# cuulee/reporter

Measured on AMD Instinct MI355X. Metric: GPS probes matched/sec (whole node), higher is better.
Workload: dtype f64; 1 GPU; c2; graph=metro, nodes=1048576, directed_edges=3527937, osmlr_segments=1361487, traces_per_gpu=10000, streams=1, device_batches=1, output_segments=1688548

## Files before the change

### reporter_amd/csrc/otr_kernels.h

```cpp
#pragma once
#include <cstddef>
#include <type_traits>

#include "otr_device.h"
#include "otr_mincode.h"
#include "otr_report.h"

#ifndef OTR_CAP1
#define OTR_CAP1 160
#endif
#ifndef OTR_LOAD1
#define OTR_LOAD1 7
#endif
#ifndef OTR_E1CAP
#define OTR_E1CAP 360
#endif
#ifndef OTR_E1LOAD
#define OTR_E1LOAD 14
#endif

namespace otr {

struct BatchDev {
  int32_t n_traces;
  const int64_t* trace_off;
  const double* lat;
  const double* lon;
  const int64_t* time;
  const float* acc;
  const uint8_t* mode;
};

__global__ void k_select_states(BatchDev b, ModeParams mp, int64_t* state_cnt, const int64_t* state_off,
                                int64_t* state_probe, int32_t* state_trace) {
  int t = blockIdx.x * blockDim.x + threadIdx.x;
  if (t >= b.n_traces) return;
  const int64_t lo = b.trace_off[t], hi = b.trace_off[t + 1];
  const MatchParams& P = mp.m[b.mode[t] < OTR_MODES ? b.mode[t] : 0];
  int64_t cnt = 0;
  int64_t base = state_off ? state_off[t] : 0;
  double la_last = 0.0, lo_last = 0.0;
  double la_n = lo < hi ? b.lat[lo] : 0.0, lo_n = lo < hi ? b.lon[lo] : 0.0;
  for (int64_t i = lo; i < hi; ++i) {
    const double la = la_n, lg = lo_n;
    if (i + 1 < hi) {
      la_n = b.lat[i + 1];
      lo_n = b.lon[i + 1];
    }
    const bool st = (i == lo || i == hi - 1) || gc_dist(la_last, lo_last, la, lg) >= P.interpolation_distance;
    if (st) {
      if (state_off) {
        state_probe[base + cnt] = i;
        state_trace[base + cnt] = t;
      }
      ++cnt;
      la_last = la;
      lo_last = lg;
    }
// ... 42 lines not shown
    const double by = (e6(pb.x) - plat) * kMetersPerDeg;
    const double dx = bx - ax, dy = by - ay;
    const double l2 = dx * dx + dy * dy;
    double t = 0.0;
    if (l2 > 0.0) {
      t = -(ax * dx + ay * dy) / l2;
      if (t < 0.0) t = 0.0;
      if (t > 1.0) t = 1.0;
    }
    const double qx = ax + t * dx, qy = ay + t * dy;
    const double d2 = qx * qx + qy * qy;
    const double sl = sqrt(l2);
    if (d2 < best) {
      best = d2;
      best_along = acc + t * sl;
      bqx = qx;
      bqy = qy;
    }
    acc = acc + sl;
    pa = pb;
  }
  *tests += k1 - k0 - 1;
  if (!(best <= r2)) return false;
  const double slat = plat + bqy / kMetersPerDeg, slon = plon + bqx / mpl;
  *sr_out = (int64_t)floor((slat - g.grid_min_lat) / g.grid_cell_deg);
  *sc_out = (int64_t)floor((slon - g.grid_min_lon) / g.grid_cell_deg);
  *d2_out = best;
  *frac_out = acc > 0.0 ? best_along / acc : 0.0;
  return true;
}

__device__ inline uint32_t wave_sum_u32(uint32_t v) {
  v += (uint32_t)__builtin_amdgcn_update_dpp(0, (int)v, 0x111, 0xf, 0xf, false);
  v += (uint32_t)__builtin_amdgcn_update_dpp(0, (int)v, 0x112, 0xf, 0xf, false);
  v += (uint32_t)__builtin_amdgcn_update_dpp(0, (int)v, 0x114, 0xf, 0xf, false);
  v += (uint32_t)__builtin_amdgcn_update_dpp(0, (int)v, 0x118, 0xf, 0xf, false);
  v += (uint32_t)__builtin_amdgcn_update_dpp(0, (int)v, 0x142, 0xa, 0xf, false);
  v += (uint32_t)__builtin_amdgcn_update_dpp(0, (int)v, 0x143, 0xc, 0xf, false);
  return (uint32_t)__builtin_amdgcn_readlane((int)v, 63);
}

__device__ inline uint32_t wave_min_u32(uint32_t v) {
  const int I = -1;
  auto mn = [](uint32_t a, int b) { return a < (uint32_t)b ? a : (uint32_t)b; };
  v = mn(v, __builtin_amdgcn_update_dpp(I, (int)v, 0x111, 0xf, 0xf, false));
  v = mn(v, __builtin_amdgcn_update_dpp(I, (int)v, 0x112, 0xf, 0xf, false));
  v = mn(v, __builtin_amdgcn_update_dpp(I, (int)v, 0x114, 0xf, 0xf, false));
  v = mn(v, __builtin_amdgcn_update_dpp(I, (int)v, 0x118, 0xf, 0xf, false));
  v = mn(v, __builtin_amdgcn_update_dpp(I, (int)v, 0x142, 0xa, 0xf, false));
  v = mn(v, __builtin_amdgcn_update_dpp(I, (int)v, 0x143, 0xc, 0xf, false));
  return (uint32_t)__builtin_amdgcn_readlane((int)v, 63);
}

template <int G>
struct Grp {
  static constexpr int GL = OTR_WAVE / G;
  __device__ static int g() { return G == 1 ? 0 : (int)threadIdx.x / GL; }
  __device__ static int gl() { return G == 1 ? (int)threadIdx.x : (int)threadIdx.x % GL; }
  __device__ static unsigned long long mine(unsigned long long m) {
    return G == 1 ? m : (m >> (GL * g())) & ((1ull << GL) - 1ull);
  }
  __device__ static int prefix(unsigned long long m) {
    if (G == 1) return prefix_count(m);
    return __popcll(mine(m) & ((1ull << gl()) - 1ull));
  }
  __device__ static int count(unsigned long long m) { return __popcll(mine(m)); }
  __device__ static int umax(int v) {
    if (G == 1) return __builtin_amdgcn_readfirstlane(v);
    if (G == 8) {
      int m = __builtin_amdgcn_readlane(v, 0);
#pragma unroll
      for (int q = 1; q < 8; ++q) {
        const int x = __builtin_amdgcn_readlane(v, q * GL);
        m = x > m ? x : m;
      }
      return m;
    }
    const int a = __builtin_amdgcn_readlane(v, 0), b = __builtin_amdgcn_readlane(v, GL);
    if (G == 2) return a > b ? a : b;
    const int c = __builtin_amdgcn_readlane(v, 2 * GL), d = __builtin_amdgcn_readlane(v, 3 * GL);
    const int ab = a > b ? a : b, cd = c > d ? c : d;
    return ab > cd ? ab : cd;
  }
  __device__ static bool all(bool v) {
    if (G == 1) return __builtin_amdgcn_readfirstlane((int)v) != 0;
    if (G == 8) {
      bool r = true;
#pragma unroll
      for (int q = 0; q < 8; ++q) r = r && __builtin_amdgcn_readlane((int)v, q * GL) != 0;
      return r;
    }
    const bool ab = __builtin_amdgcn_readlane((int)v, 0) != 0 && __builtin_amdgcn_readlane((int)v, GL) != 0;
    if (G == 2) return ab;
    return ab && __builtin_amdgcn_readlane((int)v, 2 * GL) != 0 && __builtin_amdgcn_readlane((int)v, 3 * GL) != 0;
  }
  __device__ static uint32_t min_u32(uint32_t v) {
    if (G == 1) return wave_min_u32(v);
    if (G == 8) {
#pragma unroll
      for (int o = 1; o < 8; o <<= 1) {
        const uint32_t x = (uint32_t)__shfl_xor((int)v, o, 8);
        v = x < v ? x : v;
      }
      return v;
    }
    const int I = -1;
    auto mn = [](uint32_t a, int b) { return a < (uint32_t)b ? a : (uint32_t)b; };
    v = mn(v, __builtin_amdgcn_update_dpp(I, (int)v, 0x111, 0xf, 0xf, false));
    v = mn(v, __builtin_amdgcn_update_dpp(I, (int)v, 0x112, 0xf, 0xf, false));
    v = mn(v, __builtin_amdgcn_update_dpp(I, (int)v, 0x114, 0xf, 0xf, false));
    v = mn(v, __builtin_amdgcn_update_dpp(I, (int)v, 0x118, 0xf, 0xf, false));
    if (G == 4) {
      const uint32_t a = (uint32_t)__builtin_amdgcn_readlane((int)v, 15);
      const uint32_t b = (uint32_t)__builtin_amdgcn_readlane((int)v, 31);
      const uint32_t c = (uint32_t)__builtin_amdgcn_readlane((int)v, 47);
      const uint32_t d = (uint32_t)__builtin_amdgcn_readlane((int)v, 63);
      const int q = g();
      return q == 0 ? a : (q == 1 ? b : (q == 2 ? c : d));
    }
    v = mn(v, __builtin_amdgcn_update_dpp(I, (int)v, 0x142, 0xa, 0xf, false));
    const uint32_t a = (uint32_t)__builtin_amdgcn_readlane((int)v, 31);
    const uint32_t b = (uint32_t)__builtin_amdgcn_readlane((int)v, 63);
    return g() ? b : a;
  }
};

constexpr int kWin = 16;
#ifndef OTR_CAND2_WAVES
#define OTR_CAND2_WAVES 5
#endif

template <int G>
__global__ __launch_bounds__(64) __attribute__((amdgpu_waves_per_eu(G == 2 ? OTR_CAND2_WAVES : 8, 8))) void k_candidates(
    DevGraph g, BatchDev b, ModeParams mp, int64_t n_states, const int64_t* state_probe, const int32_t* state_trace,
    CandBuf out, unsigned long long* counters) {
  using Gr = Grp<G>;
  constexpr int GL = Gr::GL;
  constexpr int LB = 2 * GL;
  __shared__ double s_d2[G][LB];
  __shared__ double s_p[G][LB];
  __shared__ uint32_t s_e[G][LB];
  __shared__ uint32_t s_bnd[G][kWin][kWin + 1];
  __shared__ uint32_t s_pre[G][kWin + 1];
  const int gi = Gr::g(), lane = Gr::gl();
  const int64_t n_units = (n_states + G - 1) / G;
  const int64_t s = xcd_remap(blockIdx.x, (n_units + 7) / 8) * G + gi;
  if (Gr::umax(s < n_states ? 1 : 0) == 0) return;
// ... 236 lines not shown
  return (m >> (GL * gi)) & ((1ull << GL) - 1ull);
}

template <int LM>
struct LabelT {
  using T = uint32_t;
  using W = uint32_t;
  static constexpr T kInf = 0xFFFFFFFFu;
  static constexpr W kNone = 0xFFFFFFFFu;
  __device__ static W label(T x) { return x; }
  __device__ static T make(W l, uint32_t) { return l; }
};
template <>
struct LabelT<1> {
  using T = unsigned long long;
  using W = uint32_t;
  static constexpr T kInf = 0xFFFFFFFFFFFFFFFFull;
  static constexpr W kNone = 0xFFFFFFFFu;
  __device__ static W label(T x) { return (uint32_t)(x >> 32); }
  __device__ static T make(W l, uint32_t e) { return ((unsigned long long)l << 32) | e; }
};
template <>
struct LabelT<2> {
  using T = unsigned long long;
  using W = unsigned long long;
  static constexpr T kInf = 0xFFFFFFFFFFFFFFFFull;
  static constexpr W kNone = 0xFFFFFFFFFFFFFFFFull;
  __device__ static W label(T x) { return x; }
  __device__ static T make(W l, uint32_t) { return l; }
};

template <class W>
struct WorkE {
  uint32_t node;
  W lab;
};


#ifndef OTR_PCAP1024
#define OTR_PCAP1024 512
#endif
#ifndef OTR_PCAP2048
#define OTR_PCAP2048 512
#endif
#ifndef OTR_PCAP448
#define OTR_PCAP448 448
#endif
#ifndef OTR_WCAP1024
#define OTR_WCAP1024 120
#endif
#ifndef OTR_WCAP4
#define OTR_WCAP4 16
#endif
template <int CAP, int LM>
struct SearchLds {
  static constexpr bool PRED = LM == 1;
  static constexpr bool MI8 = CAP >= 384 && CAP <= 1024 && !PRED;
  using MiT = typename std::conditional<MI8, uint8_t, uint16_t>::type;
  __device__ static MiT code(uint32_t m) {
    if constexpr (MI8) return mf8_of(m);
    else return mi_of(m);
  }
  __device__ static uint32_t gap(MiT c) {
    if constexpr (MI8) return mf8_gap(c);
    else return in_gap(c);
  }
  using W = typename LabelT<LM>::W;
  typename LabelT<LM>::T lab[CAP];
  uint32_t key[CAP];
  MiT mi[CAP];
  using Idx = typename std::conditional<(CAP <= 256 && !PRED), uint8_t, uint16_t>::type;
  static constexpr int WCAP = CAP <= 48 ? 8 : CAP <= 96 ? (PRED ? 20 : OTR_WCAP4) : CAP <= 160 ? 48 : (PRED ? CAP / 4 : (CAP <= 512 ? 64 : (CAP <= 1024 ? OTR_WCAP1024 : 128)));
  static constexpr int PCAP = PRED ? CAP
                                    : (CAP == 1024 ? OTR_PCAP1024 : (CAP == 2048 ? OTR_PCAP2048 : (CAP == 448 ? OTR_PCAP448 : CAP)));
  Idx pend[PCAP];
  WorkE<W> work[WCAP];
  int n_pend, n_keys, overflow;
};

constexpr uint32_t kEmpty = 0xFFFFFFFFu;

constexpr uint32_t kInq = 0x80000000u;
constexpr uint32_t kRel = 0x40000000u;
constexpr uint32_t kNodeMask = 0x0FFFFFFFu;
constexpr uint32_t kNoLabel = 0xFFFFFFFFu;
constexpr uint32_t kNoRoute = 0xFFFFFFFFu;

#ifdef OTR_STAMPS
#define OTR_STAMP(v) unsigned long long v = __builtin_amdgcn_s_memtime()
#else
#define OTR_STAMP(v) const unsigned long long v = 0
#endif

__device__ inline int64_t bound_mm_of(double bound) { return (int64_t)floor(bound * 1000.0); }
__device__ inline int64_t part_mm(double frac, uint32_t len_mm) { return (int64_t)llround(frac * (double)len_mm); }

template <int CAP>
__device__ inline uint32_t hslot(uint32_t node) {
  static_assert(CAP < (1 << 16), "table size fits the 16-bit scale");
  uint32_t p;
  asm("v_mul_u32_u24 %0, %1, %2" : "=v"(p) : "s"(0x9E3779u), "v"(node));
  const uint32_t h = (p >> 8) & 0xFFFFu;
  return __umul24(h, (uint32_t)CAP) >> 16;
}

template <int CAP, int LM>
__device__ inline int lds_find(const SearchLds<CAP, LM>& L, uint32_t node) {
  uint32_t h = hslot<CAP>(node);
  for (int probe = 0; probe < CAP; ++probe) {
    const uint32_t k = L.key[h];
    if (k == kEmpty) return -1;
    if ((k & kNodeMask) == node) return (int)h;
    h = h + 1 == (uint32_t)CAP ? 0u : h + 1;
  }
  return -1;
}

template <int CAP, int LM, bool COUNT = true>
__device__ inline int lds_insert(SearchLds<CAP, LM>& L, uint32_t node, bool* isnew) {
  uint32_t h = hslot<CAP>(node);
  for (int probe = 0; probe < CAP; ++probe) {
    const uint32_t k = atomicCAS(&L.key[h], kEmpty, node);
    if (k == kEmpty) {
      if (COUNT) atomicAdd(&L.n_keys, 1);
      *isnew = true;
      return (int)h;
    }
    if ((k & kNodeMask) == node) {
      *isnew = false;
      return (int)h;
    }
    h = h + 1 == (uint32_t)CAP ? 0u : h + 1;
  }
  L.overflow = 1;
  *isnew = false;
  return -1;
}

template <int CAP, int LM, int G = 1>
__device__ inline void search_init(SearchLds<CAP, LM>* Ls) {
  for (int q = 0; q < G; ++q) {
    SearchLds<CAP, LM>& L = Ls[q];
    for (int k = threadIdx.x; k < CAP; k += OTR_WAVE) {
      L.key[k] = kEmpty;
      L.lab[k] = LabelT<LM>::kInf;
    }
    if (threadIdx.x == 0) {
      L.n_pend = 0;
      L.n_keys = 0;
      L.overflow = 0;
    }
  }
  __syncthreads();
}

struct Pack {
  uint32_t sh;
  __device__ uint32_t tcap() const { return (1u << sh) - 1u; }
  template <class W>
  __device__ uint32_t d(W w) const { return (uint32_t)(w >> sh); }
  template <class W>
  __device__ uint32_t t(W w) const { return (uint32_t)(w & (W)tcap()); }
};
__host__ __device__ inline uint32_t pack_shift(int32_t bt) {
  if (bt < 0) return 0u;
  uint32_t sh = 0;
  while (((1u << sh) - 1u) < (uint32_t)bt + 1u) ++sh;
  return sh;
}
__host__ __device__ inline bool pack_fits(uint32_t bmm, uint32_t sh) {
  return (((uint64_t)bmm << sh) | ((1ull << sh) - 1ull)) < 0xFFFFFFFFull;
}

template <int CAP, int LM>
__device__ inline bool target_resolved(const SearchLds<CAP, LM>& L, const Pack& K, int tslot, uint32_t tpart,
                                       uint32_t gapT, uint32_t pd, uint32_t kmin, bool pend_empty) {
  const int ts = tslot < 0 ? 0 : tslot;
  const uint32_t key = L.key[ts];
  const typename LabelT<LM>::W lw = LabelT<LM>::label(L.lab[ts]);
  const int64_t lab = lw == LabelT<LM>::kNone ? INT64_MAX / 4 : (int64_t)K.d(lw);
  const int64_t next = (int64_t)kmin + (int64_t)gapT;
  const bool unreach = (lab < next ? lab : next) + (int64_t)tpart > (int64_t)pd;
  return (tslot < 0) | pend_empty | ((key & kRel) != 0u) | (lab < next) | unreach;
}

template <int CAP, int LM, bool COUNT = true>
__device__ inline int relax_one(SearchLds<CAP, LM>& L, const Pack& K, uint32_t dw, uint32_t len_mm,
                                uint32_t time_ds, uint32_t minin, typename LabelT<LM>::W pu, uint32_t edge,
                                uint32_t pd, uint32_t pt, uint32_t mode_bit, uint32_t& relaxed, uint32_t& knext,
                                bool& isnew) {
  using W = typename LabelT<LM>::W;
  isnew = false;
  if (!(((dw >> 28) & 7u) & mode_bit)) return -1;
  ++relaxed;
  const uint32_t nd = K.d(pu) + len_mm;
  if (nd > pd) return -1;
  const uint32_t tt = K.t(pu) + time_ds;
  if (tt > pt) return -1;
  const W nw = ((W)nd << K.sh) | (W)tt;
  const int sl = lds_insert<CAP, LM, COUNT>(L, dw & kAdjDstMask, &isnew);
  if (sl < 0) return -1;
  if (isnew) L.mi[sl] = SearchLds<CAP, LM>::code(minin);
  const typename LabelT<LM>::T nb = LabelT<LM>::make(nw, edge);
  const typename LabelT<LM>::T old = atomicMin(&L.lab[sl], nb);
  if (LabelT<LM>::label(nb) < LabelT<LM>::label(old)) {
    knext = nd < knext ? nd : knext;
    const uint32_t ok = atomicOr(&L.key[sl], kInq);
    if (!(ok & kInq)) return sl;
  }
  return -1;
}

template <int CAP>
__device__ inline int relax_sink(SearchLds<CAP, 0>& L, uint32_t* sink, const Pack& K, uint32_t dw, uint32_t len_mm,
                                 uint32_t time_ds, uint32_t minin, uint32_t pu, uint32_t pd, uint32_t pt,
                                 uint32_t mode_bit, uint32_t& relaxed, uint32_t& knext, bool& isnew) {
  const bool mode_ok = (((dw >> 28) & 7u) & mode_bit) != 0u;
  relaxed += mode_ok ? 1u : 0u;
  const uint32_t nd = K.d(pu) + len_mm;
  const uint32_t tt = K.t(pu) + time_ds;
  const uint32_t nw = (nd << K.sh) | tt;
  const uint32_t node = dw & kAdjDstMask;
  bool go = mode_ok && nd <= pd && tt <= pt;
  uint32_t* mine = sink + lane_id();
  const uint32_t h0 = hslot<CAP>(node);
  const uint32_t k0 = atomicCAS(go ? &L.key[h0] : mine, kEmpty, node);
  isnew = go && k0 == kEmpty;
  int sl = (go && (k0 == kEmpty || (k0 & kNodeMask) == node)) ? (int)h0 : -1;
  const bool coll = go && sl < 0;
  if (__ballot(coll) != 0ull) {
    if (coll) {
      uint32_t hh = h0;
      for (int probe = 1; probe < CAP; ++probe) {
        hh = hh + 1 == (uint32_t)CAP ? 0u : hh + 1;
        const uint32_t k = atomicCAS(&L.key[hh], kEmpty, node);
        if (k == kEmpty) {
          isnew = true;
          sl = (int)hh;
          break;
        }
        if ((k & kNodeMask) == node) {
          sl = (int)hh;
          break;
        }
      }
      if (sl < 0) L.overflow = 1;
    }
  }
  go = go && sl >= 0;
  using MiT = typename SearchLds<CAP, 0>::MiT;
  *((go && isnew) ? &L.mi[sl] : reinterpret_cast<MiT*>(mine)) = SearchLds<CAP, 0>::code(minin);
  const uint32_t old = atomicMin(go ? &L.lab[sl] : mine, nw);
  const bool imp = go && nw < old;
  knext = (imp && nd < knext) ? nd : knext;
  const uint32_t was = atomicOr(imp ? &L.key[sl] : mine, kInq);
  return (imp && !(was & kInq)) ? sl : -1;
}

struct NDump {
  const unsigned long long* in;
  unsigned long long* base;
  unsigned long long* ctr;
  uint32_t words, slots;
#ifdef OTR_FORCE_RETRY
  int stop_rounds;
#endif
};
__host__ __device__ constexpr uint32_t nd_words(int cap) { return 2u + (uint32_t)cap + ((uint32_t)cap + 1u) / 2u; }
#ifndef OTR_ND_IN_MIN
#define OTR_ND_IN_MIN 2048
#endif
#ifndef OTR_ND_OUT_MIN
#define OTR_ND_OUT_MIN 1024
#endif

template <int CAP, int LM, int G = 1, bool RIN = false, bool ROUT = false>
__device__ bool search_run(SearchLds<CAP, LM>* Ls, const DevGraph& g, const Pack& K, uint32_t mode_bit, bool active,
                           uint32_t start, uint32_t pd, uint32_t pt, uint32_t tnode, uint32_t tpart, uint32_t gapT,
                           int n_tgt, unsigned long long* settled, unsigned long long* relaxed,
                           unsigned long long* rounds, unsigned long long* stamps = nullptr, uint32_t* sink = nullptr,
                           const NDump* nd = nullptr, int* dslot = nullptr) {
  using Gr = Grp<G>;
  constexpr int kMaxKeys = (CAP <= 128 || CAP >= 256) ? (CAP * 7) / 8 : (CAP * OTR_LOAD1) / 8;
  const int gl = Gr::gl();
  using W = typename LabelT<LM>::W;
  SearchLds<CAP, LM>& L = Ls[Gr::g()];
  using Idx = typename SearchLds<CAP, LM>::Idx;
  constexpr int WCAP = SearchLds<CAP, LM>::WCAP;
  const bool timed = K.sh != 0u;
  const uint32_t* adjt = g.adj_t + (size_t)__builtin_ctz(mode_bit) * g.adj_t_stride;
  uint32_t kmin = 0;
  int npend = active ? 1 : 0;
  const bool resume = RIN && LM == 0 && active && nd->in != nullptr;
  const int nres = resume ? (int)nd->in[0] : 0;
  const int nrx = RIN ? Gr::umax(nres) : 0;
  if (RIN && nrx > 0) {
    const unsigned long long* D = nd->in;
    const uint32_t* M = (const uint32_t*)(D + 2 + nres);
    int np = 0;
    for (int base = 0; base < nrx; base += Gr::GL) {
      const int k = base + gl;
      bool pend = false;
      int sl = 0;
      if (k < nres) {
        const unsigned long long e = D[2 + k];
        const uint32_t key = (uint32_t)(e >> 32), node = key & kNodeMask;
        uint32_t h = hslot<CAP>(node);
        for (int probe = 0; probe < CAP; ++probe) {
          if (atomicCAS(&L.key[h], kEmpty, node) == kEmpty) break;
          h = h + 1 == (uint32_t)CAP ? 0u : h + 1;
        }
        sl = (int)h;
        L.key[sl] = key;
        L.lab[sl] = (typename LabelT<LM>::T)(uint32_t)e;
        L.mi[sl] = SearchLds<CAP, LM>::code(M[k]);
        pend = (key & kInq) != 0u;
      }
      const unsigned long long mp = __ballot(pend);
      if (pend && np + Gr::prefix(mp) < SearchLds<CAP, LM>::PCAP) L.pend[np + Gr::prefix(mp)] = (Idx)sl;
      np += Gr::count(mp);
    }
    if (resume && np > SearchLds<CAP, LM>::PCAP) {
      if (gl == 0) L.overflow = 1;
      np = SearchLds<CAP, LM>::PCAP;
    }
    if (resume) {
      npend = np;
      kmin = (uint32_t)D[1];
      if (gl == 0) L.n_keys = nres;
    }
  }
  if (!resume && active && gl == 0) {
    bool isnew;
    const int sl = lds_insert(L, start, &isnew);
    L.mi[sl] = 0;
    L.lab[sl] = LabelT<LM>::make(0u, kEmpty);
    L.key[sl] |= kInq;
    L.pend[0] = (Idx)sl;
  }
  __syncthreads();
  int tslot = -1;
  if (active && gl < n_tgt && tnode != kEmpty) {
    bool isnew;
    tslot = lds_insert(L, tnode, &isnew);
    if (tslot >= 0 && isnew) L.mi[tslot] = SearchLds<CAP, LM>::code(gapT);
  }
  __syncthreads();
  uint32_t my_settled = 0, my_relaxed = 0, my_rounds = 0;
  unsigned long long cyc[4] = {0, 0, 0, 0};
  bool done = !active, grew = false;
#ifdef OTR_FORCE_RETRY
  int force_round = 0;
#endif
  int nkeys = 0;
  for (;;) {
    OTR_STAMP(t0);
    const int np = done ? 0 : npend;
    OTR_STAMP(t1);
    const bool res = done | (gl >= n_tgt) | target_resolved(L, K, tslot, tpart, gapT, pd, kmin, np == 0);
    done = done || Gr::mine(__ballot(!res)) == 0ull || np == 0;
    OTR_STAMP(t2);
    cyc[0] += t1 - t0;
    cyc[1] += t2 - t1;
    if (Gr::all(done)) break;
    if (!done && gl == 0) ++my_rounds;
    uint32_t knext = 0xFFFFFFFFu;
    int kept = 0, nw = 0;
    const int npx = Gr::umax(np);
    for (int base = 0; base < npx; base += Gr::GL) {
      const int k = base + gl;
      const bool in = k < np;
      const int sl = in ? (int)L.pend[k] : 0;
      const W lb = LabelT<LM>::label(L.lab[sl]);
      const uint32_t key = L.key[sl];
      const uint32_t d = K.d(lb);
      bool take = in && (uint64_t)d < (uint64_t)kmin + SearchLds<CAP, LM>::gap(L.mi[sl]);
      take = take && nw + Gr::prefix(__ballot(take)) < WCAP;
      const unsigned long long mt = __ballot(take), mk = __ballot(in && !take);
      __syncthreads();
      if (take) {
        const uint32_t node = key & kNodeMask;
        L.work[nw + Gr::prefix(mt)] = WorkE<W>{node, lb};
        L.key[sl] = node | kRel;
      }
      const bool keep = in && !take;
      if (keep) L.pend[kept + Gr::prefix(mk)] = (Idx)sl;
      knext = (keep && d < knext) ? d : knext;
      nw += Gr::count(mt);
      kept += Gr::count(mk);
      __syncthreads();
    }
    npend = kept;
    OTR_STAMP(t3);
    cyc[2] += t3 - t2;
    const int nwx = Gr::umax(4 * nw);
    uint32_t tail = 0u;
    for (int base = 0; base < nwx; base += Gr::GL) {
      const int k = base + gl;
      int psl = -1;
      bool isnew = false;
      if (k < 4 * nw) {
        const WorkE<W> wk = L.work[k >> 2];
        const uint32_t wnode = wk.node;
        const int slot = k & 3;
        if (slot == 0) ++my_settled;
        const uint32_t tq = adjt[4 * (size_t)wnode + slot];
        const uint4 r = ld16(g.adj + 4 * (size_t)wnode + slot);
        const uint32_t tt = timed ? tq : 0u;
        if constexpr (LM == 0) {
#ifdef OTR_NO_SINK
          psl = relax_one<CAP, LM, false>(L, K, r.x & ~kAdjMore, r.y, tt, r.z, wk.lab, 0u, pd, pt, mode_bit,
                                          my_relaxed, knext, isnew);
#else
          psl = relax_sink<CAP>(L, sink, K, r.x & ~kAdjMore, r.y, tt, r.z, wk.lab, pd, pt, mode_bit, my_relaxed,
                                knext, isnew);
#endif
        } else {
          const uint32_t e0 = LM == 1 ? g.node_row[wnode] : 0u;
          psl = relax_one<CAP, LM, false>(L, K, r.x & ~kAdjMore, r.y, tt, r.z, wk.lab, e0 + slot, pd, pt, mode_bit,
                                          my_relaxed, knext, isnew);
        }
        tail |= slot == 3 ? (r.x & kAdjMore) : 0u;
      }
      nkeys += Gr::count(__ballot(isnew));
      const unsigned long long mp = __ballot(psl >= 0);
#ifndef OTR_NO_SINK
      if constexpr (LM == 0 && G == 1) {
        const int p = npend + Gr::prefix(mp);
        constexpr int PC = SearchLds<CAP, LM>::PCAP;
        *(psl >= 0 ? &L.pend[p < PC ? p : PC - 1] : reinterpret_cast<Idx*>(sink + lane_id())) = (Idx)psl;
      } else
#endif
      if (psl >= 0) {
        const int p = npend + Gr::prefix(mp);
        L.pend[p < SearchLds<CAP, LM>::PCAP ? p : SearchLds<CAP, LM>::PCAP - 1] = (Idx)psl;
      }
      npend += Gr::count(mp);
    }
    if (SearchLds<CAP, LM>::PCAP < CAP && npend > SearchLds<CAP, LM>::PCAP) {
      if (gl == 0) L.overflow = 1;
      npend = SearchLds<CAP, LM>::PCAP;
    }
    if (__ballot(tail != 0u) != 0ull) {
      if (gl == 0) L.n_pend = npend;
      __syncthreads();
      for (int base = 0; base < nwx; base += Gr::GL) {
        const int k = base + gl;
        if (k < 4 * nw && (k & 3) == 3) {
          const WorkE<W> wk = L.work[k >> 2];
          const uint32_t wnode = wk.node;
          if (g.adj[4 * (size_t)wnode + 3].x & kAdjMore)
            for (uint32_t e = g.node_row[wnode] + 4; e < g.node_row[wnode + 1]; ++e) {
              const uint4 pk = ld16(g.edge_pack + e);
              const uint32_t tt = timed ? g.et(__builtin_ctz(mode_bit))[e] : 0u;
              bool isnew;
              const int psl = relax_one(L, K, pk.x | ((pk.z & 7u) << 28), pk.y, tt, pk.w, wk.lab, e, pd, pt, mode_bit,
                                        my_relaxed, knext, isnew);
              if (psl >= 0) {
                const int p = atomicAdd(&L.n_pend, 1);
                if (p < SearchLds<CAP, LM>::PCAP) L.pend[p] = (Idx)psl;
                else L.overflow = 1;
              }
            }
        }
      }
      __syncthreads();
      npend = L.n_pend;
      if (npend > SearchLds<CAP, LM>::PCAP) npend = SearchLds<CAP, LM>::PCAP;
    }
    __syncthreads();
    OTR_STAMP(t4);
    cyc[3] += t4 - t3;
    const uint32_t km = Gr::min_u32(knext);
    if (!done) kmin = km;
    const int keys = L.n_keys + nkeys;
    if (!done && (L.overflow || keys > kMaxKeys)) {
      grew = !L.overflow && keys > kMaxKeys;
      done = true;
    }
#ifdef OTR_FORCE_RETRY
    ++force_round;
    if (ROUT && !done && nd->base != nullptr && nd->stop_rounds > 0 && force_round >= nd->stop_rounds &&
        !L.overflow) {
      grew = true;
      done = true;
    }
#endif
    __syncthreads();
    if (done && active && gl == 0 && (keys > kMaxKeys || grew)) L.overflow = 1;
  }
  if (gl == 0) L.n_keys += nkeys;
  if (ROUT) *dslot = -1;
  if (ROUT && LM == 0 && __ballot(grew && active && nd->base != nullptr) != 0ull) {
    int v = 0;
    if (grew && active && nd->base != nullptr && gl == 0) v = (int)atomicAdd(nd->ctr, 1ull);
    v = __shfl(v, 0, Gr::GL);
    const bool dump = grew && active && nd->base != nullptr && (uint32_t)v < nd->slots;
    unsigned long long* D = dump ? nd->base + (size_t)v * nd->words : nullptr;
    int n = 0;
    for (int base = 0; base < CAP; base += Gr::GL) {
      const int k = base + gl;
      const uint32_t key = (dump && k < CAP) ? L.key[k] : kEmpty;
      const bool has = key != kEmpty;
      const unsigned long long m = __ballot(has);
      if (has) D[2 + n + Gr::prefix(m)] = (unsigned long long)(uint32_t)L.lab[k] | ((unsigned long long)key << 32);
      n += Gr::count(m);
    }
    uint32_t* M = dump ? (uint32_t*)(D + 2 + n) : nullptr;
    int q = 0;
    for (int base = 0; base < CAP; base += Gr::GL) {
      const int k = base + gl;
      const bool has = dump && k < CAP && L.key[k] != kEmpty;
      const unsigned long long m = __ballot(has);
      if (has) M[q + Gr::prefix(m)] = SearchLds<CAP, LM>::gap(L.mi[k]);
      q += Gr::count(m);
    }
    if (dump && gl == 0) {
      D[0] = (unsigned long long)(uint32_t)n;
      D[1] = kmin;
    }
    *dslot = dump ? v : -1;
  }
#ifdef OTR_STAMPS
  if (stamps && threadIdx.x == 0)
    for (int q = 0; q < 4; ++q) atomicAdd(&stamps[q * kCShards + cshard()], cyc[q]);
#endif
  if (settled) *settled += my_settled;
  if (relaxed) *relaxed += my_relaxed;
  if (rounds) *rounds += my_rounds;
  __syncthreads();
  return !L.overflow;
}

struct PrepArgs {
  int64_t n_states;
  const int64_t* prev;
  const double* bound;
  const int32_t* cand_count;
  const uint32_t* cand_edge;
  const double* cand_p;
  const int32_t* state_trace;
  const uint8_t* mode;
  uint4* cprep;
  uint2* cprep_t;
  uint2* clen;
  int32_t* nroot;
  uint32_t turn_modes;
};

template <int G>
__global__ __launch_bounds__(256) void k_prep(DevGraph g, PrepArgs a) {
  constexpr int GL = OTR_WAVE / G;
  const int64_t s = ((int64_t)blockIdx.x * (blockDim.x / OTR_WAVE) + threadIdx.x / OTR_WAVE) * G +
                    (threadIdx.x % OTR_WAVE) / GL;
  const int lane = threadIdx.x % GL;
  if (s >= a.n_states) return;
  const int K = a.cand_count[s];
  if (K <= 0) return;
// ... 185 lines not shown
  const int32_t bt = a.bt[s];
  const uint32_t sh = pack_shift(bt);
#ifdef OTR_FORCE_GENERAL
  const bool general = true;
#else
  const bool general = !pack_fits(bmm, sh) || turn;
#endif
  uint32_t pre = 0u;
  if (a.est_first_keys > 0 && !general && !turn && !a.forced[s]) {
    float reach = (float)bmm * 1e-3f;
    if (bt >= 0) reach = fminf(reach, (float)bt * 0.1f * a.est_v[md]);
    const float est = a.est_k * reach * reach;
    if (est > (float)a.est_first_keys) {
      uint32_t st = 0;
      while ((int)st + 1 < a.n_tiers && (float)a.tier_keys[st] < est) ++st;
      pre = 1u | (st << 1);
    }
  }
  const uint32_t meta = (uint32_t)a.cand_count[s] | ((uint32_t)md << 8) | ((a.forced[s] ? 1u : 0u) << 10) |
                        (sh << 11) | ((general ? 1u : 0u) << 16) | (turn << 17) | (pre << 18);
  const int64_t to = a.trans_off[s];
  if (turn && a.flag_turn) a.flag_turn[o] = 5;
  a.rec[3 * o] = make_uint4((uint32_t)s, (uint32_t)sp, root, bmm);
  a.rec[3 * o + 1] = make_uint4(d0min, meta, (uint32_t)same, (uint32_t)(same >> 32));
  a.rec[3 * o + 2] = make_uint4(0u, (uint32_t)bt, (uint32_t)to, (uint32_t)((uint64_t)to >> 32));
}

#ifndef OTR_ROUTE2_WAVES
#define OTR_ROUTE2_WAVES 8
#endif

__device__ inline int nth_set_bit(unsigned long long m, int q) {
  for (int j = 0; j < q; ++j) m &= m - 1;
  return __ffsll((long long)m) - 1;
}

template <int CAP, int G, bool LIST, bool WIDE = false, bool CNT = true>
__device__ __forceinline__ void route_unit(const DevGraph& gr, const RouteArgs& a, unsigned long long* counters,
                                           SearchLds<CAP, WIDE ? 2 : 0>* Ls, int64_t w, int64_t n_tasks,
                                           uint32_t* sink, uint4 (*trec)[3]) {
  constexpr int LM = WIDE ? 2 : 0;
  using Gr = Grp<G>;
  const int lane = Gr::gl();
  const int64_t tw = (LIST ? 0 : a.task_base) + w * G + Gr::g();
  const bool have = tw < n_tasks;
  const int64_t task = have ? (LIST ? a.task_list[tw] : tw) : 0;
  OTR_STAMP(ts_in);
  bool search, fits, forced;
  int start_tier = -1;
  uint32_t tnode = kEmpty, tpart = 0, gapT = 1, d0min = 0xFFFFFFFFu, root = 0, bmm = 0, mode_bit = 1;
  uint32_t pd = 0, pt = 0xFFFFFFFFu;
  int Kb;
  Pack K;
  {
    const uint4 r0 = have ? a.rec[3 * task] : make_uint4(0u, 0u, 0u, 0u);
    const uint4 r1 = have ? a.rec[3 * task + 1] : make_uint4(0xFFFFFFFFu, 0u, 0u, 0u);
    const uint4 r2 = have ? a.rec[3 * task + 2] : make_uint4(0u, 0u, 0u, 0u);
    if (lane == 0) {
      trec[Gr::g()][0] = r0;
      trec[Gr::g()][1] = r1;
      trec[Gr::g()][2] = r2;
    }
    const int64_t s = r0.x;
    const unsigned long long mask = ((unsigned long long)r1.w << 32) | r1.z;
    const int64_t sp = r0.y;
    Kb = (int)(r1.y & 0xFFu);
    K.sh = (r1.y >> 11) & 31u;
    const bool general = (r1.y >> 16) & 1u;
    fits = Kb <= Gr::GL && (WIDE || !general) && !((r1.y >> 17) & 1u);
    const bool pre = G >= 2 && !LIST && have && ((r1.y >> 18) & 1u);
    if (pre) {
      start_tier = (int)((r1.y >> 19) & 7u);
      fits = false;
    }
    mode_bit = 1u << ((r1.y >> 8) & 3u);
    bmm = r0.w;
    root = r0.z;
    d0min = r1.x;
    const int32_t bt = (int32_t)r2.y;
    uint32_t ej = 0;
    double pj = 0;
    bool needed = false;
    uint4 cq = make_uint4(0u, 0u, 0u, 0u);
    if (have && !pre && lane < Kb) {
      ej = a.cand_edge[s * OTR_KMAX + lane];
      pj = a.cand_p[s * OTR_KMAX + lane];
      cq = a.cprep[s * OTR_KMAX + lane];
      tpart = cq.x;
    }
    const int nsrc = have && !pre ? __popcll(mask) : 0;
    const int iq = lane < nsrc ? nth_set_bit(mask, lane) : 0;
    uint32_t e_q = 0, t_q = 0;
    double p_q = 0;
    if (lane < nsrc) {
      e_q = a.cand_edge[sp * OTR_KMAX + iq];
      p_q = a.cand_p[sp * OTR_KMAX + iq];
      if (bt >= 0) t_q = a.cprep_t[sp * OTR_KMAX + iq].y;
    }
    for (int q = 0; q < nsrc; ++q) {
      uint32_t ei;
      double pi;
      if (q < Gr::GL) {
        ei = (uint32_t)__shfl((int)e_q, q, Gr::GL);
        pi = __shfl(p_q, q, Gr::GL);
      } else {
        const int i = nth_set_bit(mask, q);
        ei = a.cand_edge[sp * OTR_KMAX + i];
        pi = a.cand_p[sp * OTR_KMAX + i];
      }
      if (lane < Kb && !(ej == ei && pj >= pi)) needed = true;
    }
    const uint32_t t0 = (uint32_t)__shfl((int)t_q, 0, Gr::GL);
    bool feasible_root = d0min <= bmm;
    pd = feasible_root ? bmm - d0min : 0u;
    if (bt >= 0) {
      feasible_root = feasible_root && t0 <= (uint32_t)bt;
      pt = t0 <= (uint32_t)bt ? (uint32_t)bt - t0 : 0u;
    }
    forced = have && ((r1.y >> 10) & 1u);
    const unsigned long long need_mask = __ballot(needed);
    search = have && fits && !forced && feasible_root && Gr::mine(need_mask) != 0ull;
    if (needed) {
      tnode = cq.y;
      gapT = cq.z ? cq.z : 1u;
    }
  }
  unsigned long long settled = 0, relaxed = 0, rounds = 0;
  OTR_STAMP(ts_set);
  NDump nd{};
  int dslot = -1;
  constexpr bool kIn = LIST && !WIDE && CAP >= OTR_ND_IN_MIN, kOut = LIST && !WIDE && CAP >= OTR_ND_OUT_MIN;
  constexpr bool kDumps = kIn || kOut;
  if (kIn) {
    const int32_t rs = (a.dump_in != nullptr && search) ? a.task_dump[task] : -1;
    nd.in = rs >= 0 ? a.dump_in + (size_t)rs * a.dump_in_words : nullptr;
  }
  if (kOut) {
    nd.base = a.dump_out;
    nd.ctr = a.dump_ctr;
    nd.words = a.dump_out_words;
    nd.slots = a.dump_out_slots;
#ifdef OTR_FORCE_RETRY
    nd.stop_rounds = (a.force_edge >> 7) & 1 ? 2 + Gr::g() : 0;
#endif
  }
  search_init<CAP, LM, G>(Ls);
  bool ok = search_run<CAP, LM, G, kIn, kOut>(Ls, gr, K, mode_bit, search, root, pd, pt, tnode, tpart, gapT, Kb, &settled,
                                   &relaxed, &rounds, counters ? counters + 16 * kCShards : nullptr, sink,
                                   kDumps ? &nd : nullptr, kDumps ? &dslot : nullptr) &&
            fits;
#ifdef OTR_FORCE_RETRY
  if (G >= 2 && !LIST) ok = false;
#endif
  OTR_STAMP(ts_srch);
  SearchLds<CAP, LM>& L = Ls[Gr::g()];
  int64_t lab = -1;
  if (ok && search && tnode != kEmpty && !forced) {
    const int sl = lds_find(L, tnode);
    if (sl >= 0 && LabelT<LM>::label(L.lab[sl]) != LabelT<LM>::kNone) lab = (int64_t)LabelT<LM>::label(L.lab[sl]);
  }
  asm volatile("" ::: "memory");
  uint32_t ntr = 0;
  if (have && forced && Kb > Gr::GL) {
    const uint4 r1 = trec[Gr::g()][1], r2 = trec[Gr::g()][2];
    const unsigned long long mask = ((unsigned long long)r1.w << 32) | r1.z;
    uint32_t* trow = a.trans + (int64_t)(((uint64_t)r2.w << 32) | r2.z);
    for (int q = 0; q < __popcll(mask); ++q) {
      const int i = nth_set_bit(mask, q);
      for (int j = lane; j < Kb; j += Gr::GL) trow[(int64_t)i * Kb + j] = kNoRoute;
    }
  } else if (have && (ok || forced)) {
    const uint4 r0 = trec[Gr::g()][0], r1 = trec[Gr::g()][1], r2 = trec[Gr::g()][2];
    const int64_t s = r0.x;
    const unsigned long long mask = ((unsigned long long)r1.w << 32) | r1.z;
    if (search) ntr = (uint32_t)Kb * (uint32_t)__popcll(mask);
    const int64_t sp = r0.y;
    const int32_t bt = (int32_t)r2.y;
    uint32_t* trow = a.trans + (int64_t)(((uint64_t)r2.w << 32) | r2.z);
    const int nsrc = __popcll(mask);
    const int iq = lane < nsrc ? nth_set_bit(mask, lane) : 0;
    uint32_t e_q = 0, w_q = 0, t_q = 0;
    uint2 l_q = make_uint2(0u, 0u);
    double p_q = 0;
    if (lane < nsrc) {
      e_q = a.cand_edge[sp * OTR_KMAX + iq];
      p_q = a.cand_p[sp * OTR_KMAX + iq];
      w_q = a.cprep[sp * OTR_KMAX + iq].w;
      if (bt >= 0) t_q = a.cprep_t[sp * OTR_KMAX + iq].y;
      l_q = a.clen[sp * OTR_KMAX + iq];
    }
    uint32_t ej = 0, tpt = 0;
    double pj = 0;
    if (lane < Kb) {
      ej = a.cand_edge[s * OTR_KMAX + lane];
      pj = a.cand_p[s * OTR_KMAX + lane];
      tpt = bt >= 0 ? a.cprep_t[s * OTR_KMAX + lane].x : 0u;
    }
    for (int q = 0; q < nsrc; ++q) {
      int i;
      uint32_t ei, wi, ti, li, lti;
      double pi;
      if (q < Gr::GL) {
        i = __shfl(iq, q, Gr::GL);
        ei = (uint32_t)__shfl((int)e_q, q, Gr::GL);
        pi = __shfl(p_q, q, Gr::GL);
        wi = (uint32_t)__shfl((int)w_q, q, Gr::GL);
        ti = (uint32_t)__shfl((int)t_q, q, Gr::GL);
        li = (uint32_t)__shfl((int)l_q.x, q, Gr::GL);
        lti = (uint32_t)__shfl((int)l_q.y, q, Gr::GL);
      } else {
        i = nth_set_bit(mask, q);
        ei = a.cand_edge[sp * OTR_KMAX + i];
        pi = a.cand_p[sp * OTR_KMAX + i];
        wi = a.cprep[sp * OTR_KMAX + i].w;
        ti = bt >= 0 ? a.cprep_t[sp * OTR_KMAX + i].y : 0u;
        const uint2 l = a.clen[sp * OTR_KMAX + i];
        li = l.x;
        lti = l.y;
      }
      if (lane < Kb) {
        int64_t r = -1, rt = 0;
        if (forced) {
          r = -1;
        } else if (ej == ei && pj >= pi) {
          r = part_mm(pj - pi, li);
          if (bt >= 0) rt = part_mm(pj - pi, lti);
        } else if (lab >= 0) {
          r = (int64_t)wi + K.d((uint64_t)lab) + tpart;
          if (bt >= 0) rt = (int64_t)ti + K.t((uint64_t)lab) + tpt;
        }
        const bool valid = r >= 0 && r <= (int64_t)bmm && (bt < 0 || rt <= (int64_t)bt);
        trow[(int64_t)i * Kb + lane] = valid ? (uint32_t)r : kNoRoute;
      }
    }
  }
  if (have && !ok && !forced && lane == 0) {
    const uint32_t meta = a.rec[3 * task + 1].y;
    const bool general = ((meta >> 16) & 1u) != 0u, turn = ((meta >> 17) & 1u) != 0u;
#ifdef OTR_FORCE_GENERAL
    a.overflow_flag[task] = 3;
#else
    if (!turn) a.overflow_flag[task] = general ? 3 : (start_tier >= 0 ? 16 + start_tier : 1);
#endif
    if (!WIDE && !turn && a.task_dump != nullptr) a.task_dump[task] = dslot;
  }
#ifdef OTR_STAMPS
  if (G == 2 && counters && threadIdx.x == 0) {
    OTR_STAMP(ts_out);
// ... 1175 lines not shown
```

Baseline: 34.98 million probes/s.

## Drop pending-bit atomics, vectorize LDS init, use ballot loop bounds in search rounds

For group sizes other than 8, the search drops the atomicOr on the pending bit and instead treats a slot as newly pending when its previous label was infinite. The LDS table is cleared with 16-byte stores over the lab/key region, and round loops end on a ballot instead of a cross-group max via readlane. Final-distance tests use 32-bit wraparound comparisons instead of 64-bit math, and candidate loads are kept from the prologue rather than reloaded in the transition writer. The dump path rebuilds the pending bit so resume stays consistent. The risk is subtle correctness around the label-infinity test for re-enqueue and the 32-bit overflow handling.

After: 36.09 million probes/s (median of 6 runs). +3.2%, better.

```diff
diff --git a/reporter_amd/csrc/otr_kernels.h b/reporter_amd/csrc/otr_kernels.h
--- a/reporter_amd/csrc/otr_kernels.h
+++ b/reporter_amd/csrc/otr_kernels.h
@@ -4,6 +4,7 @@
 
 #include "otr_device.h"
 #include "otr_mincode.h"
+#include "otr_pred.h"
 #include "otr_report.h"
 
 #ifndef OTR_CAP1
@@ -152,6 +153,8 @@
   return (uint32_t)__builtin_amdgcn_readlane((int)v, 63);
 }
 
+__host__ __device__ constexpr bool old_rounds(int g) { return g == 8; }
+
 template <int G>
 struct Grp {
   static constexpr int GL = OTR_WAVE / G;
@@ -183,16 +186,13 @@
     return ab > cd ? ab : cd;
   }
   __device__ static bool all(bool v) {
-    if (G == 1) return __builtin_amdgcn_readfirstlane((int)v) != 0;
     if (G == 8) {
       bool r = true;
 #pragma unroll
       for (int q = 0; q < 8; ++q) r = r && __builtin_amdgcn_readlane((int)v, q * GL) != 0;
       return r;
     }
-    const bool ab = __builtin_amdgcn_readlane((int)v, 0) != 0 && __builtin_amdgcn_readlane((int)v, GL) != 0;
-    if (G == 2) return ab;
-    return ab && __builtin_amdgcn_readlane((int)v, 2 * GL) != 0 && __builtin_amdgcn_readlane((int)v, 3 * GL) != 0;
+    return __ballot(!v) == 0ull;
   }
   __device__ static uint32_t min_u32(uint32_t v) {
     if (G == 1) return wave_min_u32(v);
@@ -535,8 +535,9 @@
 #ifndef OTR_WCAP4
 #define OTR_WCAP4 16
 #endif
+__host__ __device__ constexpr int search_lds_align(int cap, int lm) { return cap <= 48 ? (lm == 0 ? 4 : 8) : 16; }
 template <int CAP, int LM>
-struct SearchLds {
+struct alignas(search_lds_align(CAP, LM)) SearchLds {
   static constexpr bool PRED = LM == 1;
   static constexpr bool MI8 = CAP >= 384 && CAP <= 1024 && !PRED;
   using MiT = typename std::conditional<MI8, uint8_t, uint16_t>::type;
@@ -622,11 +623,23 @@
 
 template <int CAP, int LM, int G = 1>
 __device__ inline void search_init(SearchLds<CAP, LM>* Ls) {
+  using S = SearchLds<CAP, LM>;
+  constexpr size_t kFill = (sizeof(typename LabelT<LM>::T) + sizeof(uint32_t)) * CAP;
+  static_assert(offsetof(S, lab) == 0 && offsetof(S, key) == sizeof(typename LabelT<LM>::T) * CAP,
+                "lab[] and key[] lead the table, back to back");
+  static_assert(LabelT<LM>::kInf == (typename LabelT<LM>::T)~0ull && kEmpty == 0xFFFFFFFFu, "all-ones fill");
+  static_assert(old_rounds(G) || (kFill % 16 == 0 && sizeof(S) % 16 == 0 && alignof(S) % 16 == 0),
+                "the fill region and the tables' stride are whole 16-byte words");
   for (int q = 0; q < G; ++q) {
     SearchLds<CAP, LM>& L = Ls[q];
-    for (int k = threadIdx.x; k < CAP; k += OTR_WAVE) {
-      L.key[k] = kEmpty;
-      L.lab[k] = LabelT<LM>::kInf;
+    if constexpr (old_rounds(G)) {
+      for (int k = threadIdx.x; k < CAP; k += OTR_WAVE) {
+        L.key[k] = kEmpty;
+        L.lab[k] = LabelT<LM>::kInf;
+      }
+    } else {
+      uint4* p = reinterpret_cast<uint4*>(&L);
+      for (int k = threadIdx.x; k < (int)(kFill / 16); k += OTR_WAVE) p[k] = make_uint4(kEmpty, kEmpty, kEmpty, kEmpty);
     }
     if (threadIdx.x == 0) {
       L.n_pend = 0;
@@ -655,19 +668,24 @@
   return (((uint64_t)bmm << sh) | ((1ull << sh) - 1ull)) < 0xFFFFFFFFull;
 }
 
-template <int CAP, int LM>
+template <int CAP, int LM, bool OLD = false>
 __device__ inline bool target_resolved(const SearchLds<CAP, LM>& L, const Pack& K, int tslot, uint32_t tpart,
                                        uint32_t gapT, uint32_t pd, uint32_t kmin, bool pend_empty) {
   const int ts = tslot < 0 ? 0 : tslot;
   const uint32_t key = L.key[ts];
   const typename LabelT<LM>::W lw = LabelT<LM>::label(L.lab[ts]);
-  const int64_t lab = lw == LabelT<LM>::kNone ? INT64_MAX / 4 : (int64_t)K.d(lw);
-  const int64_t next = (int64_t)kmin + (int64_t)gapT;
-  const bool unreach = (lab < next ? lab : next) + (int64_t)tpart > (int64_t)pd;
-  return (tslot < 0) | pend_empty | ((key & kRel) != 0u) | (lab < next) | unreach;
-}
-
-template <int CAP, int LM, bool COUNT = true>
+  if constexpr (LM != 2 && !OLD) {
+    const bool fin = target_final32(lw == LabelT<LM>::kNone, K.d(lw), kmin, gapT, tpart, pd);
+    return (tslot < 0) | pend_empty | ((key & kRel) != 0u) | fin;
+  } else {
+    const int64_t lab = lw == LabelT<LM>::kNone ? INT64_MAX / 4 : (int64_t)K.d(lw);
+    const int64_t next = (int64_t)kmin + (int64_t)gapT;
+    const bool unreach = (lab < next ? lab : next) + (int64_t)tpart > (int64_t)pd;
+    return (tslot < 0) | pend_empty | ((key & kRel) != 0u) | (lab < next) | unreach;
+  }
+}
+
+template <int CAP, int LM, bool COUNT = true, bool OLD = false>
 __device__ inline int relax_one(SearchLds<CAP, LM>& L, const Pack& K, uint32_t dw, uint32_t len_mm,
                                 uint32_t time_ds, uint32_t minin, typename LabelT<LM>::W pu, uint32_t edge,
                                 uint32_t pd, uint32_t pt, uint32_t mode_bit, uint32_t& relaxed, uint32_t& knext,
@@ -688,13 +706,17 @@
   const typename LabelT<LM>::T old = atomicMin(&L.lab[sl], nb);
   if (LabelT<LM>::label(nb) < LabelT<LM>::label(old)) {
     knext = nd < knext ? nd : knext;
-    const uint32_t ok = atomicOr(&L.key[sl], kInq);
-    if (!(ok & kInq)) return sl;
+    if constexpr (OLD) {
+      const uint32_t ok = atomicOr(&L.key[sl], kInq);
+      if (!(ok & kInq)) return sl;
+    } else {
+      if (old == LabelT<LM>::kInf) return sl;
+    }
   }
   return -1;
 }
 
-template <int CAP>
+template <int CAP, bool OLD = false>
 __device__ inline int relax_sink(SearchLds<CAP, 0>& L, uint32_t* sink, const Pack& K, uint32_t dw, uint32_t len_mm,
                                  uint32_t time_ds, uint32_t minin, uint32_t pu, uint32_t pd, uint32_t pt,
                                  uint32_t mode_bit, uint32_t& relaxed, uint32_t& knext, bool& isnew) {
@@ -736,8 +758,12 @@
   const uint32_t old = atomicMin(go ? &L.lab[sl] : mine, nw);
   const bool imp = go && nw < old;
   knext = (imp && nd < knext) ? nd : knext;
-  const uint32_t was = atomicOr(imp ? &L.key[sl] : mine, kInq);
-  return (imp && !(was & kInq)) ? sl : -1;
+  if constexpr (OLD) {
+    const uint32_t was = atomicOr(imp ? &L.key[sl] : mine, kInq);
+    return (imp && !(was & kInq)) ? sl : -1;
+  } else {
+    return (imp && old == kNoLabel) ? sl : -1;
+  }
 }
 
 struct NDump {
@@ -764,6 +790,8 @@
                            unsigned long long* rounds, unsigned long long* stamps = nullptr, uint32_t* sink = nullptr,
                            const NDump* nd = nullptr, int* dslot = nullptr) {
   using Gr = Grp<G>;
+  constexpr bool OLD = old_rounds(G);
+  static_assert(!(OLD && (RIN || ROUT)), "the dump and resume code assumes keys without the pending bit");
   constexpr int kMaxKeys = (CAP <= 128 || CAP >= 256) ? (CAP * 7) / 8 : (CAP * OTR_LOAD1) / 8;
   const int gl = Gr::gl();
   using W = typename LabelT<LM>::W;
@@ -794,7 +822,7 @@
           h = h + 1 == (uint32_t)CAP ? 0u : h + 1;
         }
         sl = (int)h;
-        L.key[sl] = key;
+        L.key[sl] = key & ~kInq;
         L.lab[sl] = (typename LabelT<LM>::T)(uint32_t)e;
         L.mi[sl] = SearchLds<CAP, LM>::code(M[k]);
         pend = (key & kInq) != 0u;
@@ -818,7 +846,7 @@
     const int sl = lds_insert(L, start, &isnew);
     L.mi[sl] = 0;
     L.lab[sl] = LabelT<LM>::make(0u, kEmpty);
-    L.key[sl] |= kInq;
+    if (OLD) L.key[sl] |= kInq;
     L.pend[0] = (Idx)sl;
   }
   __syncthreads();
@@ -840,7 +868,8 @@
     OTR_STAMP(t0);
     const int np = done ? 0 : npend;
     OTR_STAMP(t1);
-    const bool res = done | (gl >= n_tgt) | target_resolved(L, K, tslot, tpart, gapT, pd, kmin, np == 0);
+    const bool res =
+        done | (gl >= n_tgt) | target_resolved<CAP, LM, OLD>(L, K, tslot, tpart, gapT, pd, kmin, np == 0);
     done = done || Gr::mine(__ballot(!res)) == 0ull || np == 0;
     OTR_STAMP(t2);
     cyc[0] += t1 - t0;
@@ -849,24 +878,32 @@
     if (!done && gl == 0) ++my_rounds;
     uint32_t knext = 0xFFFFFFFFu;
     int kept = 0, nw = 0;
-    const int npx = Gr::umax(np);
-    for (int base = 0; base < npx; base += Gr::GL) {
+    const int npx = OLD ? Gr::umax(np) : 0;
+    for (int base = 0; OLD ? base < npx : __ballot(base + gl < np) != 0ull; base += Gr::GL) {
       const int k = base + gl;
       const bool in = k < np;
       const int sl = in ? (int)L.pend[k] : 0;
       const W lb = LabelT<LM>::label(L.lab[sl]);
       const uint32_t key = L.key[sl];
       const uint32_t d = K.d(lb);
-      bool take = in && (uint64_t)d < (uint64_t)kmin + SearchLds<CAP, LM>::gap(L.mi[sl]);
-      take = take && nw + Gr::prefix(__ballot(take)) < WCAP;
-      const unsigned long long mt = __ballot(take), mk = __ballot(in && !take);
+      bool take, keep;
+      if constexpr (OLD) {
+        take = in && (uint64_t)d < (uint64_t)kmin + SearchLds<CAP, LM>::gap(L.mi[sl]);
+        take = take && nw + Gr::prefix(__ballot(take)) < WCAP;
+        keep = in && !take;
+      } else {
+        const uint32_t gp = SearchLds<CAP, LM>::gap(L.mi[sl]);
+        if constexpr (LM != 2) take = in & in_final32(d, kmin, gp);
+        else take = in & ((uint64_t)d < (uint64_t)kmin + gp);
+        take = take & (nw + Gr::prefix(__ballot(take)) < WCAP);
+        keep = in & !take;
+      }
+      const unsigned long long mt = __ballot(take), mk = __ballot(keep);
       __syncthreads();
       if (take) {
-        const uint32_t node = key & kNodeMask;
-        L.work[nw + Gr::prefix(mt)] = WorkE<W>{node, lb};
-        L.key[sl] = node | kRel;
-      }
-      const bool keep = in && !take;
+        L.work[nw + Gr::prefix(mt)] = WorkE<W>{key & kNodeMask, lb};
+        L.key[sl] = (key & kNodeMask) | kRel;
+      }
       if (keep) L.pend[kept + Gr::prefix(mk)] = (Idx)sl;
       knext = (keep && d < knext) ? d : knext;
       nw += Gr::count(mt);
@@ -876,9 +913,9 @@
     npend = kept;
     OTR_STAMP(t3);
     cyc[2] += t3 - t2;
-    const int nwx = Gr::umax(4 * nw);
     uint32_t tail = 0u;
-    for (int base = 0; base < nwx; base += Gr::GL) {
+    const int nwx = OLD ? Gr::umax(4 * nw) : 0;
+    for (int base = 0; OLD ? base < nwx : __ballot(base + gl < 4 * nw) != 0ull; base += Gr::GL) {
       const int k = base + gl;
       int psl = -1;
       bool isnew = false;
@@ -892,16 +929,16 @@
         const uint32_t tt = timed ? tq : 0u;
         if constexpr (LM == 0) {
 #ifdef OTR_NO_SINK
-          psl = relax_one<CAP, LM, false>(L, K, r.x & ~kAdjMore, r.y, tt, r.z, wk.lab, 0u, pd, pt, mode_bit,
-                                          my_relaxed, knext, isnew);
+          psl = relax_one<CAP, LM, false, OLD>(L, K, r.x & ~kAdjMore, r.y, tt, r.z, wk.lab, 0u, pd, pt, mode_bit,
+                                               my_relaxed, knext, isnew);
 #else
-          psl = relax_sink<CAP>(L, sink, K, r.x & ~kAdjMore, r.y, tt, r.z, wk.lab, pd, pt, mode_bit, my_relaxed,
-                                knext, isnew);
+          psl = relax_sink<CAP, OLD>(L, sink, K, r.x & ~kAdjMore, r.y, tt, r.z, wk.lab, pd, pt, mode_bit, my_relaxed,
+                                     knext, isnew);
 #endif
         } else {
           const uint32_t e0 = LM == 1 ? g.node_row[wnode] : 0u;
-          psl = relax_one<CAP, LM, false>(L, K, r.x & ~kAdjMore, r.y, tt, r.z, wk.lab, e0 + slot, pd, pt, mode_bit,
-                                          my_relaxed, knext, isnew);
+          psl = relax_one<CAP, LM, false, OLD>(L, K, r.x & ~kAdjMore, r.y, tt, r.z, wk.lab, e0 + slot, pd, pt,
+                                               mode_bit, my_relaxed, knext, isnew);
         }
         tail |= slot == 3 ? (r.x & kAdjMore) : 0u;
       }
@@ -927,7 +964,7 @@
     if (__ballot(tail != 0u) != 0ull) {
       if (gl == 0) L.n_pend = npend;
       __syncthreads();
-      for (int base = 0; base < nwx; base += Gr::GL) {
+      for (int base = 0; OLD ? base < nwx : __ballot(base + gl < 4 * nw) != 0ull; base += Gr::GL) {
         const int k = base + gl;
         if (k < 4 * nw && (k & 3) == 3) {
           const WorkE<W> wk = L.work[k >> 2];
@@ -937,8 +974,8 @@
               const uint4 pk = ld16(g.edge_pack + e);
               const uint32_t tt = timed ? g.et(__builtin_ctz(mode_bit))[e] : 0u;
               bool isnew;
-              const int psl = relax_one(L, K, pk.x | ((pk.z & 7u) << 28), pk.y, tt, pk.w, wk.lab, e, pd, pt, mode_bit,
-                                        my_relaxed, knext, isnew);
+              const int psl = relax_one<CAP, LM, true, OLD>(L, K, pk.x | ((pk.z & 7u) << 28), pk.y, tt, pk.w, wk.lab, e,
+                                                            pd, pt, mode_bit, my_relaxed, knext, isnew);
               if (psl >= 0) {
                 const int p = atomicAdd(&L.n_pend, 1);
                 if (p < SearchLds<CAP, LM>::PCAP) L.pend[p] = (Idx)psl;
@@ -986,7 +1023,11 @@
       const uint32_t key = (dump && k < CAP) ? L.key[k] : kEmpty;
       const bool has = key != kEmpty;
       const unsigned long long m = __ballot(has);
-      if (has) D[2 + n + Gr::prefix(m)] = (unsigned long long)(uint32_t)L.lab[k] | ((unsigned long long)key << 32);
+      if (has) {
+        const uint32_t lb = (uint32_t)L.lab[k];
+        const uint32_t kq = (lb != kNoLabel && !(key & kRel)) ? key | kInq : key;
+        D[2 + n + Gr::prefix(m)] = (unsigned long long)lb | ((unsigned long long)kq << 32);
+      }
       n += Gr::count(m);
     }
     uint32_t* M = dump ? (uint32_t*)(D + 2 + n) : nullptr;
@@ -1278,6 +1319,10 @@
   uint32_t pd = 0, pt = 0xFFFFFFFFu;
   int Kb;
   Pack K;
+  uint32_t ej = 0, e_q = 0, t_q = 0;
+  double pj = 0, p_q = 0;
+  int iq = 0;
+  constexpr bool kKeep = !LIST && !CNT && !old_rounds(G);
   {
     const uint4 r0 = have ? a.rec[3 * task] : make_uint4(0u, 0u, 0u, 0u);
     const uint4 r1 = have ? a.rec[3 * task + 1] : make_uint4(0xFFFFFFFFu, 0u, 0u, 0u);
@@ -1304,8 +1349,6 @@
     root = r0.z;
     d0min = r1.x;
     const int32_t bt = (int32_t)r2.y;
-    uint32_t ej = 0;
-    double pj = 0;
     bool needed = false;
     uint4 cq = make_uint4(0u, 0u, 0u, 0u);
     if (have && !pre && lane < Kb) {
@@ -1315,9 +1358,7 @@
       tpart = cq.x;
     }
     const int nsrc = have && !pre ? __popcll(mask) : 0;
-    const int iq = lane < nsrc ? nth_set_bit(mask, lane) : 0;
-    uint32_t e_q = 0, t_q = 0;
-    double p_q = 0;
+    iq = lane < nsrc ? nth_set_bit(mask, lane) : 0;
     if (lane < nsrc) {
       e_q = a.cand_edge[sp * OTR_KMAX + iq];
       p_q = a.cand_p[sp * OTR_KMAX + iq];
@@ -1404,22 +1445,30 @@
     const int32_t bt = (int32_t)r2.y;
     uint32_t* trow = a.trans + (int64_t)(((uint64_t)r2.w << 32) | r2.z);
     const int nsrc = __popcll(mask);
-    const int iq = lane < nsrc ? nth_set_bit(mask, lane) : 0;
-    uint32_t e_q = 0, w_q = 0, t_q = 0;
+    uint32_t w_q = 0;
     uint2 l_q = make_uint2(0u, 0u);
-    double p_q = 0;
+    if (!kKeep) {
+      if (!LIST) {
+        e_q = t_q = ej = 0u;
+        p_q = pj = 0.0;
+      }
+      iq = lane < nsrc ? nth_set_bit(mask, lane) : 0;
+    }
     if (lane < nsrc) {
-      e_q = a.cand_edge[sp * OTR_KMAX + iq];
-      p_q = a.cand_p[sp * OTR_KMAX + iq];
+      if (!kKeep) {
+        e_q = a.cand_edge[sp * OTR_KMAX + iq];
+        p_q = a.cand_p[sp * OTR_KMAX + iq];
+        if (bt >= 0) t_q = a.cprep_t[sp * OTR_KMAX + iq].y;
+      }
       w_q = a.cprep[sp * OTR_KMAX + iq].w;
-      if (bt >= 0) t_q = a.cprep_t[sp * OTR_KMAX + iq].y;
       l_q = a.clen[sp * OTR_KMAX + iq];
     }
-    uint32_t ej = 0, tpt = 0;
-    double pj = 0;
+    uint32_t tpt = 0;
     if (lane < Kb) {
-      ej = a.cand_edge[s * OTR_KMAX + lane];
-      pj = a.cand_p[s * OTR_KMAX + lane];
+      if (!kKeep) {
+        ej = a.cand_edge[s * OTR_KMAX + lane];
+        pj = a.cand_p[s * OTR_KMAX + lane];
+      }
       tpt = bt >= 0 ? a.cprep_t[s * OTR_KMAX + lane].x : 0u;
     }
     for (int q = 0; q < nsrc; ++q) {
diff --git a/reporter_amd/csrc/otr_pred.h b/reporter_amd/csrc/otr_pred.h
--- /dev/null
+++ b/reporter_amd/csrc/otr_pred.h
@@ -0,0 +1,20 @@
+#pragma once
+#include <hip/hip_runtime.h>
+
+#include <cstdint>
+
+namespace otr {
+
+__host__ __device__ inline bool in_final32(uint32_t d, uint32_t kmin, uint32_t gap) { return d - kmin < gap; }
+
+__host__ __device__ inline bool target_final32(bool none, uint32_t d, uint32_t kmin, uint32_t gapT, uint32_t tpart,
+                                               uint32_t pd) {
+  const uint32_t next = kmin + gapT;
+  const bool carry = next < kmin;
+  const bool below = !none & (carry | (d < next));
+  const uint32_t m = below ? d : next;
+  const bool unreach = (!below & carry) | (tpart > pd) | (m > pd - tpart);
+  return below | unreach;
+}
+
+}
```
